# yaricom/Plastic-UNet

Hardware: AMD Instinct MI355X
Metric: training images/sec (128x128, bs=32 per GPU) (higher is better)
Workload: dtype f32; 1 GPU; C2: UNetp depth 5 base_ch 64, oja rule, 1x128x128, fwd+BCE+bwd+Adam; global_batch=32, per_gpu_batch=32, img=128, parallelism=single, step_launch=eager

## Files before the change

### plastic-unet_amd/csrc/common.h

```cpp
#pragma once

#include <hip/hip_runtime.h>
#include <stdint.h>
#include <stdio.h>
#include <stdarg.h>
#include <type_traits>

#include "plastic_unet.h"

namespace pu {

extern thread_local char g_last_error[512];

inline int fail(int code, const char* fmt, ...) {
    va_list ap;
    va_start(ap, fmt);
    vsnprintf(g_last_error, sizeof(g_last_error), fmt, ap);
    va_end(ap);
    return code;
}

inline int check_launch(const char* what) {
    hipError_t e = hipGetLastError();
    if (e != hipSuccess) return fail(PU_ERR_LAUNCH, "%s: %s", what, hipGetErrorString(e));
// ... 76 lines not shown
    return (xcd < r ? xcd * (q + 1) : r * (q + 1) + (xcd - r) * q) + local;
}


template <int N, typename F, int I = 0>
__device__ __forceinline__ void static_for(F&& f) {
    if constexpr (I < N) {
        f(std::integral_constant<int, I>{});
        static_for<N, F, I + 1>(static_cast<F&&>(f));
    }
}
constexpr unsigned LEAN_OOB = 0x80000000u;
typedef __attribute__((address_space(3))) void lds_void_t;

__device__ __forceinline__ void lean_load(const void* base, unsigned bytes, void* lds_dst, unsigned voff, unsigned soff) {
    const unsigned long long b = (unsigned long long)base;
    const unsigned lo = __builtin_amdgcn_readfirstlane((unsigned)b);
    const unsigned hi = __builtin_amdgcn_readfirstlane((unsigned)(b >> 32));
    void* ub = (void*)(((unsigned long long)hi << 32) | lo);
    __amdgpu_buffer_rsrc_t r = __builtin_amdgcn_make_buffer_rsrc(ub, 0, (int)__builtin_amdgcn_readfirstlane(bytes), 0x00020000);
    __builtin_amdgcn_raw_ptr_buffer_load_lds(r, (lds_void_t*)lds_dst, 16, voff, __builtin_amdgcn_readfirstlane(soff), 0, 0);
}

}
```

### plastic-unet_amd/csrc/conv_common.h

```cpp
#pragma once
#include "common.h"

namespace pu {

typedef float f32x4 __attribute__((ext_vector_type(4)));
typedef float f32x16 __attribute__((ext_vector_type(16)));

struct IgemmParams {
    int M, N, K, k_pad;
    int Hi, Wi, Ho, Wo, kh, kw, stride, pad;
    int C, c0, c1;
    const float* src0;
    const float* src1;
    const float* wt;
    const float* bias;
    float* dst0;
    float* dst1;
    const float* mask0;
    const float* mask1;
    int n0, flags;
    int cgroup, taps, gn;
    int vec_epi;
    int ksplit, t_per;
    float* part;
// ... 11 lines not shown
    int oh0, ow0;
    int b;
};

__device__ __forceinline__ EpiRow epi_row(const IgemmParams& p, int m) {
    if (!(p.flags & PU_EPI_SHUFFLE2)) return {m, 0, 0, p.cscale ? (int)fdiv(m, p.dHW) : 0};
    const int t2 = fdiv(m, p.dWo);
    const int wo = m - t2 * p.Wo;
    const int bb = fdiv(t2, p.dHo);
    const int ho = t2 - bb * p.Ho;
    return {(long long)bb * p.shuf_h, 2 * ho - p.shuf_off, 2 * wo - p.shuf_off, bb};
}

__device__ __forceinline__ bool shuf_off(const IgemmParams& p, const EpiRow& r, int n, long long* off, int* c) {
    const int co = p.N >> 2;
    const int ij = fdiv(n, p.dCo);
    *c = n - ij * co;
    const int oh = r.oh0 + (ij >> 1), ow = r.ow0 + (ij & 1);
    if ((unsigned)oh >= (unsigned)p.shuf_h || (unsigned)ow >= (unsigned)p.shuf_w) return false;
    *off = ((r.pix + oh) * p.shuf_w + ow) * co + *c;
    return true;
}

__device__ __forceinline__ void epi_store4(const IgemmParams& p, const EpiRow& r, int n, f32x4 v) {
    float* dst;
    const float* msk;
    long long off;
    int nb;
    const long long pix = r.pix;
    if (p.flags & PU_EPI_SHUFFLE2) {
        if (!shuf_off(p, r, n, &off, &nb)) return;
        dst = p.dst0; msk = p.mask0;
    } else if (n < p.n0) {
        off = pix * p.n0 + n;
        dst = p.dst0; msk = p.mask0; nb = n;
    } else {
        off = pix * (p.N - p.n0) + (n - p.n0);
        dst = p.dst1; msk = p.mask1; nb = n;
    }
    if (p.bias) v += *reinterpret_cast<const f32x4*>(p.bias + nb);
    if (p.resid) v += *reinterpret_cast<const f32x4*>(p.resid + off);
    if (p.flags & PU_EPI_RELU) {
#pragma unroll
        for (int e = 0; e < 4; ++e) v[e] = fmaxf(v[e], 0.f);
    }
    if (msk) {
        const f32x4 mv = *reinterpret_cast<const f32x4*>(msk + off);
#pragma unroll
        for (int e = 0; e < 4; ++e) if (!(mv[e] > 0.f)) v[e] = 0.f;
    }
    if (p.cscale) v *= *reinterpret_cast<const f32x4*>(p.cscale + (long long)r.b * p.cs_ld + nb);
    if (p.flags & PU_EPI_ACCUM) v += *reinterpret_cast<const f32x4*>(dst + off);
    *reinterpret_cast<f32x4*>(dst + off) = v;
}

typedef __bf16 bf16x8_t __attribute__((ext_vector_type(8)));

typedef float f32x2 __attribute__((ext_vector_type(2)));
typedef __bf16 bf16x2_t __attribute__((ext_vector_type(2)));

__device__ __forceinline__ unsigned pk_bf16(f32x2 v) {
    const bf16x2_t h = __builtin_convertvector(v, bf16x2_t);
    return __builtin_bit_cast(unsigned, h);
}

__device__ __forceinline__ void split3_pairs(const f32x4 lo4, const f32x4 hi4, bf16x8_t& h, bf16x8_t& m, bf16x8_t& l) {
#pragma clang fp contract(off)
    typedef unsigned u32x4 __attribute__((ext_vector_type(4)));
    u32x4 hv, mv, lv;
#pragma unroll
    for (int q = 0; q < 4; ++q) {
        const f32x2 x = q < 2 ? f32x2{lo4[2 * q], lo4[2 * q + 1]} : f32x2{hi4[2 * q - 4], hi4[2 * q - 3]};
        const unsigned a = pk_bf16(x);
        const f32x2 af = {__builtin_bit_cast(float, a << 16), __builtin_bit_cast(float, a & 0xffff0000u)};
        const f32x2 r = x - af;
        const unsigned b = pk_bf16(r);
// ... 20 lines not shown
```

### plastic-unet_amd/csrc/elementwise.hip

```cpp
#include "common.h"

#include <math.h>

namespace pu {

typedef float f32x4 __attribute__((ext_vector_type(4)));
typedef __bf16 bf16x4 __attribute__((ext_vector_type(4)));

template <typename T> __device__ __forceinline__ f32x4 ld4(const T* p);
template <> __device__ __forceinline__ f32x4 ld4<float>(const float* p) { return *reinterpret_cast<const f32x4*>(p); }
template <> __device__ __forceinline__ f32x4 ld4<__bf16>(const __bf16* p) {
    const bf16x4 v = *reinterpret_cast<const bf16x4*>(p);
    return f32x4{(float)v[0], (float)v[1], (float)v[2], (float)v[3]};
}
template <typename T> __device__ __forceinline__ void st4(T* p, f32x4 v);
template <> __device__ __forceinline__ void st4<float>(float* p, f32x4 v) { *reinterpret_cast<f32x4*>(p) = v; }
template <> __device__ __forceinline__ void st4<__bf16>(__bf16* p, f32x4 v) {
    *reinterpret_cast<bf16x4*>(p) = bf16x4{(__bf16)v[0], (__bf16)v[1], (__bf16)v[2], (__bf16)v[3]};
}

__device__ __forceinline__ int ungroup_k(int k, int C, int taps, int G) {
    if (G == 0 || k >= taps * C) return k;
    const int tg = k / G, cg = k - tg * G;
    const int g = tg / taps, tap = tg - g * taps;
    return tap * C + g * G + cg;
}

__device__ __forceinline__ float pack_value(const float* __restrict__ w, int mode, int d0, int d1, int taps,
                                            int row, int kc, int G) {
    const int Ck = (mode == PU_PACK_CONV_DGRAD) ? d0 : d1;
    const int k = (mode == PU_PACK_CONVT_FWD) ? kc : ungroup_k(kc, Ck, taps, G);
    float v = 0.f;
    if (mode == PU_PACK_CONV_FWD) {
        if (k < taps * d1) {
            int tap = k / d1, i = k - tap * d1;
            v = w[((long long)row * d1 + i) * taps + tap];
        }
    } else if (mode == PU_PACK_CONV_DGRAD) {
        if (k < taps * d0) {
            int tapf = k / d0, o = k - tapf * d0;
            int tap = taps - 1 - tapf;
// ... 226 lines not shown
    }
}

template <typename T>
struct Vec16 {
    static constexpr int V = 16 / sizeof(T);
    float v[V];
};
template <typename T>
__device__ __forceinline__ Vec16<T> ld16(const T* p) {
    Vec16<T> r;
    if constexpr (sizeof(T) == 4) {
        const f32x4 a = *reinterpret_cast<const f32x4*>(p);
#pragma unroll
        for (int e = 0; e < 4; ++e) r.v[e] = a[e];
    } else {
        typedef __bf16 b8 __attribute__((ext_vector_type(8)));
        const b8 a = *reinterpret_cast<const b8*>(p);
#pragma unroll
        for (int e = 0; e < 8; ++e) r.v[e] = (float)a[e];
    }
    return r;
}
template <typename T>
__device__ __forceinline__ void st16(T* p, const float (&v)[Vec16<T>::V]) {
    if constexpr (sizeof(T) == 4) {
        *reinterpret_cast<f32x4*>(p) = f32x4{v[0], v[1], v[2], v[3]};
    } else {
        typedef __bf16 b8 __attribute__((ext_vector_type(8)));
        b8 a;
#pragma unroll
        for (int e = 0; e < 8; ++e) a[e] = (__bf16)v[e];
        *reinterpret_cast<b8*>(p) = a;
    }
}

template <typename T>
__global__ void maxpool_fwd_win_kernel(const T* __restrict__ x, T* __restrict__ y, int W, int C, int Ho, int Wo,
                                       long long total, const float* __restrict__ scale) {
    constexpr int V = Vec16<T>::V;
    const int CV = C / V;
    for (long long idx = blockIdx.x * (long long)blockDim.x + threadIdx.x; idx < total;
         idx += (long long)gridDim.x * blockDim.x) {
        const int cv = int(idx % CV);
        long long t = idx / CV;
        const int wo = int(t % Wo); t /= Wo;
        const int ho = int(t % Ho);
        const long long b = t / Ho;
        const long long base = (b * 2 * Ho + 2 * ho) * (long long)W + 2 * wo;
        float best[V];
// ... 35 lines not shown
        for (int e = 0; e < V; ++e) { best[e] = -INFINITY; arg[e] = 0; }
#pragma unroll
        for (int q = 0; q < 4; ++q) {
            xv[q] = ld16(x + (base + (q >> 1) * W + (q & 1)) * C + cv * V);
#pragma unroll
            for (int e = 0; e < V; ++e) pool_take(xv[q].v[e], q, best[e], arg[e]);
        }
        Vec16<T> g = ld16(dy + idx * V);
        if (scale) {
#pragma unroll
            for (int e = 0; e < V; ++e) g.v[e] *= scale[b * C + cv * V + e];
        }
#pragma unroll
        for (int q = 0; q < 4; ++q) {
            T* d = dx + (base + (q >> 1) * W + (q & 1)) * C + cv * V;
            float out[V];
#pragma unroll
            for (int e = 0; e < V; ++e) out[e] = (arg[e] == q && (!relu_mask || xv[q].v[e] > 0.f)) ? g.v[e] : 0.f;
            if (accumulate) {
                const Vec16<T> o = ld16(d);
#pragma unroll
                for (int e = 0; e < V; ++e) out[e] = o.v[e] + out[e];
            }
            st16(d, out);
        }
    }
}

template <typename T = float>
__global__ void outconv_fwd_kernel(const T* __restrict__ x, const float* __restrict__ w, const float* __restrict__ b,
                                   float* __restrict__ y, long long rows, int C) {
    const int lane16 = threadIdx.x & 15;
    const long long groups = (long long)gridDim.x * (blockDim.x >> 4);
    const float bias = b ? b[0] : 0.f;
    for (long long m = blockIdx.x * (long long)(blockDim.x >> 4) + (threadIdx.x >> 4); m < rows + 0; m += groups) {
        float s = 0.f;
        for (int c = lane16 * 4; c < C; c += 64) {
            f32x4 v = ld4(x + m * C + c);
            f32x4 ww = *reinterpret_cast<const f32x4*>(w + c);
            s += dot4_fma(v, ww);
        }
        s += __shfl_xor(s, 8, 16);
        s += __shfl_xor(s, 4, 16);
        s += __shfl_xor(s, 2, 16);
        s += __shfl_xor(s, 1, 16);
        if (lane16 == 0) y[m] = s + bias;
    }
// ... 11 lines not shown
constexpr int OC_BLOCKS = 1024;

template <typename T = float>
__global__ void outconv_bwd_kernel(const T* __restrict__ x, const float* __restrict__ w, const float* __restrict__ dy,
                                   T* __restrict__ dx, float* __restrict__ partial, long long rows, int C,
                                   int relu_mask) {
    __shared__ float red[16][65];
    __shared__ float redb[16];
    const int lane16 = threadIdx.x & 15;
    const int grp = threadIdx.x >> 4;
    float* out = partial + (long long)blockIdx.x * (C + 1);
    for (int j = 0; j * 64 < C; ++j) {
        const int c = lane16 * 4 + 64 * j;
        float a0 = 0.f, a1 = 0.f, a2 = 0.f, a3 = 0.f, ab = 0.f;
        for (long long m = blockIdx.x * 16LL + grp; m < rows; m += (long long)gridDim.x * 16) {
            const float g = dy[m];
            ab += g;
            if (c < C) {
                f32x4 v = ld4(x + m * C + c);
                f32x4 ww = *reinterpret_cast<const f32x4*>(w + c);
                f32x4 o;
#pragma unroll
                for (int e = 0; e < 4; ++e) o[e] = (!relu_mask || v[e] > 0.f) ? g * ww[e] : 0.f;
                st4(dx + m * C + c, o);
                a0 += g * v[0]; a1 += g * v[1]; a2 += g * v[2]; a3 += g * v[3];
            }
        }
        __syncthreads();
        red[grp][lane16 * 4 + 0] = a0;
        red[grp][lane16 * 4 + 1] = a1;
        red[grp][lane16 * 4 + 2] = a2;
        red[grp][lane16 * 4 + 3] = a3;
        if (lane16 == 0) redb[grp] = ab;
        __syncthreads();
        const int t = threadIdx.x;
        if (t < 64 && 64 * j + t < C) {
            float s = 0.f;
            for (int q = 0; q < 16; ++q) s += red[q][t];
            out[64 * j + t] = s;
        }
        if (j == 0 && t == 64) {
            float s = 0.f;
            for (int q = 0; q < 16; ++q) s += redb[q];
            out[C] = s;
        }
    }
}
// ... 9 lines not shown
    __shared__ float redb[P];
    const int lane = threadIdx.x % L, grp = threadIdx.x / L;
    const int c = 4 * lane;
    const f32x4 ww = *reinterpret_cast<const f32x4*>(w + c);
    float a0 = 0.f, a1 = 0.f, a2 = 0.f, a3 = 0.f, ab = 0.f;
    const long long stride = (long long)gridDim.x * P;
    for (long long m0 = blockIdx.x * (long long)P + grp; m0 < rows; m0 += OCN_U * stride) {
        f32x4 v[OCN_U];
        float g[OCN_U];
#pragma unroll
        for (int u = 0; u < OCN_U; ++u) {
            const long long m = m0 + u * stride;
            const bool ok = m < rows;
            g[u] = ok ? dy[m] : 0.f;
            v[u] = ok ? ld4(x + m * C + c) : f32x4{0.f, 0.f, 0.f, 0.f};
        }
#pragma unroll
        for (int u = 0; u < OCN_U; ++u) {
            const long long m = m0 + u * stride;
            if (m < rows) {
                f32x4 o;
#pragma unroll
                for (int e = 0; e < 4; ++e) o[e] = (!relu_mask || v[u][e] > 0.f) ? g[u] * ww[e] : 0.f;
                st4(dx + m * C + c, o);
                ab += g[u];
                a0 += g[u] * v[u][0]; a1 += g[u] * v[u][1]; a2 += g[u] * v[u][2]; a3 += g[u] * v[u][3];
            }
        }
    }
    red[grp][c + 0] = a0;
    red[grp][c + 1] = a1;
    red[grp][c + 2] = a2;
    red[grp][c + 3] = a3;
    if (lane == 0) redb[grp] = ab;
    __syncthreads();
    float* out = partial + (long long)blockIdx.x * (C + 1);
    const int t = threadIdx.x;
    if (t < C) {
        float s = 0.f;
        for (int q = 0; q < P; ++q) s += red[q][t];
        out[t] = s;
    } else if (t == C) {
        float s = 0.f;
        for (int q = 0; q < P; ++q) s += redb[q];
        out[C] = s;
    }
}
// ... 524 lines not shown
```

### plastic-unet_amd/csrc/igemm.hip

```cpp
#include "conv_common.h"
#include <type_traits>

namespace pu {


constexpr int IG_BK = 16;
constexpr int IG_LDS = IG_BK + 4;

enum { LOAD_CHUNK16 = 0, LOAD_VEC4 = 1, LOAD_SCALAR = 2 };


template <int MODE>
__device__ __forceinline__ f32x4 load_a4(const IgemmParams& p, int pb, int hb, int wb, int k) {
    f32x4 v = {0.f, 0.f, 0.f, 0.f};
    if (MODE == LOAD_SCALAR) {
#pragma unroll
        for (int e = 0; e < 4; ++e) {
            int ke = k + e;
            if (ke < p.K) {
                int tap = fdiv(ke, p.dC);
                int c = ke - tap * p.C;
                int r = fdiv(tap, p.dKw);
                int s = tap - r * p.kw;
                int hi = hb + r, wi = wb + s;
// ... 3 lines not shown
                }
            }
        }
        return v;
    } else {
        if (k < p.K) {
            int tap = fdiv(k, p.dC);
            int c = k - tap * p.C;
            int r = fdiv(tap, p.dKw);
            int s = tap - r * p.kw;
            int hi = hb + r, wi = wb + s;
            if ((unsigned)hi < (unsigned)p.Hi && (unsigned)wi < (unsigned)p.Wi) {
                long long pix = (long long)pb + hi * p.Wi + wi;
                const float* src = c < p.c0 ? p.src0 + pix * p.c0 + c : p.src1 + pix * p.c1 + (c - p.c0);
                v = *reinterpret_cast<const f32x4*>(src);
            }
        }
        return v;
    }
}


typedef unsigned u32x4_t __attribute__((ext_vector_type(4)));
__device__ __forceinline__ __amdgpu_buffer_rsrc_t epi_rsrc(const void* base, bool on) {
    const unsigned long long b = (unsigned long long)base;
    const unsigned lo = __builtin_amdgcn_readfirstlane((unsigned)b);
    const unsigned hi = __builtin_amdgcn_readfirstlane((unsigned)(b >> 32));
    void* ub = (void*)(((unsigned long long)hi << 32) | lo);
    return __builtin_amdgcn_make_buffer_rsrc(ub, 0, on ? 0x7fffffff : 0, 0x00020000);
}

template <bool MASK, int FM, int FN>
__device__ __forceinline__ void epilogue_batched(const IgemmParams& p, f32x16 (&acc)[FM][FN], int m0, int nc0, int lr,
                                                 int lh) {
    const bool relu = p.flags & PU_EPI_RELU;
    const int n1 = p.N - p.n0;
    unsigned orow[FM][FN];
    bool first[FN];
#pragma unroll
    for (int j = 0; j < FN; ++j) first[j] = nc0 + j * 32 < p.n0;
#pragma unroll
    for (int i = 0; i < FM; ++i) {
        const int m = m0 + i * 32 + lr;
#pragma unroll
        for (int j = 0; j < FN; ++j) {
            const int c = nc0 + j * 32 + 4 * lh - (first[j] ? 0 : p.n0);
// ... 21 lines not shown
    }
#pragma unroll
    for (int j = 0; j < FN; ++j) {
        const __amdgpu_buffer_rsrc_t rd = epi_rsrc(first[j] ? p.dst0 : p.dst1, true);
        const bool has_mk = (first[j] ? p.mask0 : p.mask1) != nullptr;
#pragma unroll
        for (int i = 0; i < FM; ++i)
#pragma unroll
            for (int q = 0; q < 4; ++q) {
                f32x4 v;
#pragma unroll
                for (int e = 0; e < 4; ++e) v[e] = acc[i][j][4 * q + e];
                if constexpr (!MASK) v += ov[0][j][q];
                if (relu) {
#pragma unroll
                    for (int e = 0; e < 4; ++e) v[e] = fmaxf(v[e], 0.f);
                }
                if constexpr (MASK) {
                    if (has_mk) {
#pragma unroll
                        for (int e = 0; e < 4; ++e) if (!(ov[i][j][q][e] > 0.f)) v[e] = 0.f;
                    }
                }
                __builtin_amdgcn_raw_buffer_store_b128(__builtin_bit_cast(u32x4_t, v), rd, orow[i][j], 32 * q, 0);
            }
    }
}

template <int FM, int FN>
__device__ __forceinline__ void epilogue_batched_shuf(const IgemmParams& p, f32x16 (&acc)[FM][FN], int m0, int nc0,
                                                      int lr, int lh) {
    const bool relu = p.flags & PU_EPI_RELU;
    const int co = p.N >> 2;
    unsigned orow[FM][FN];
    int cj[FN];
#pragma unroll
    for (int j = 0; j < FN; ++j) {
        const int nj = nc0 + j * 32;
        const int ij = nj < p.N ? nj / co : 0;
        cj[j] = nj - ij * co + 4 * lh;
#pragma unroll
        for (int i = 0; i < FM; ++i) {
            const int m = m0 + i * 32 + lr;
            unsigned o = LEAN_OOB;
            if (m < p.M && nj < p.N) {
                const int t2 = fdiv(m, p.dWo);
                const int wo = m - t2 * p.Wo;
// ... 8 lines not shown
    f32x4 bv[FN][4];
    const __amdgpu_buffer_rsrc_t rb = epi_rsrc(p.bias, true);
#pragma unroll
    for (int j = 0; j < FN; ++j)
#pragma unroll
        for (int q = 0; q < 4; ++q)
            bv[j][q] = __builtin_bit_cast(f32x4, __builtin_amdgcn_raw_buffer_load_b128(
                rb, nc0 + j * 32 < p.N ? (unsigned)cj[j] * 4u : LEAN_OOB, 32 * q, 0));
    const __amdgpu_buffer_rsrc_t rd = epi_rsrc(p.dst0, true);
#pragma unroll
    for (int j = 0; j < FN; ++j)
#pragma unroll
        for (int i = 0; i < FM; ++i)
#pragma unroll
            for (int q = 0; q < 4; ++q) {
                f32x4 v;
#pragma unroll
                for (int e = 0; e < 4; ++e) v[e] = acc[i][j][4 * q + e];
                v += bv[j][q];
                if (relu) {
#pragma unroll
                    for (int e = 0; e < 4; ++e) v[e] = fmaxf(v[e], 0.f);
                }
                __builtin_amdgcn_raw_buffer_store_b128(__builtin_bit_cast(u32x4_t, v), rd, orow[i][j], 32 * q, 0);
            }
}

template <int BM, int BN, int WM, int WN, bool BATCH = false>
__device__ __forceinline__ void epilogue(const IgemmParams& p, f32x16 (&acc)[BM / WM / 32][BN / WN / 32], int m_blk,
                                         int n_blk, int wm, int wn, int lr, int lh) {
    constexpr int FM = BM / WM / 32;
    constexpr int FN = BN / WN / 32;
    if constexpr (BATCH) {
        if (p.vec_epi && !(p.flags & (PU_EPI_SHUFFLE2 | PU_EPI_ACCUM)) && !p.resid && !p.cscale && p.n0 % 32 == 0 &&
            p.N % 32 == 0 && (long long)p.M * p.N < (1LL << 29)) {
            const int m0 = m_blk + wm * (BM / WM), nc0 = n_blk + wn * (BN / WN);
            if ((p.mask0 || p.mask1) && !p.bias) {
                epilogue_batched<true, FM, FN>(p, acc, m0, nc0, lr, lh);
                return;
            }
            if (!p.mask0 && !p.mask1 && p.bias) {
                epilogue_batched<false, FM, FN>(p, acc, m0, nc0, lr, lh);
                return;
            }
        }
        if (p.vec_epi && (p.flags & PU_EPI_SHUFFLE2) && !(p.flags & PU_EPI_ACCUM) && !p.resid && !p.cscale && p.bias &&
            !p.mask0 && p.shuf_off == 0 && p.shuf_h == 2 * p.Ho && p.shuf_w == 2 * p.Wo && (p.N / 4) % 32 == 0 &&
// ... 349 lines not shown
        }
        __builtin_amdgcn_sched_group_barrier(0x100, 2 * (FM + FN), 0);
        __builtin_amdgcn_sched_group_barrier(0x008, 8 * FM * FN, 0);
    }
    asm volatile("s_waitcnt vmcnt(0)" ::: "memory");
    if (p.ksplit == 1) {
        epilogue<BM, BN, WM, WN>(p, acc, m_blk, n_blk, wm, wn, lr, lh);
        return;
    }
    float* part = p.part + (long long)kz * p.M * p.N;
#pragma unroll
    for (int i = 0; i < FM; ++i) {
        const int m = m_blk + wm * (BM / WM) + i * 32 + lr;
        if (m >= p.M) continue;
#pragma unroll
        for (int j = 0; j < FN; ++j)
#pragma unroll
            for (int q = 0; q < 4; ++q) {
                const int n = n_blk + wn * (BN / WN) + j * 32 + 8 * q + 4 * lh;
                if (n >= p.N) continue;
                f32x4 v;
#pragma unroll
                for (int e = 0; e < 4; ++e) v[e] = acc[i][j][4 * q + e];
                *reinterpret_cast<f32x4*>(part + (long long)m * p.N + n) = v;
            }
    }
}


__device__ __forceinline__ void split3_bf16(const f32x4 lo4, const f32x4 hi4, bf16x8_t& h, bf16x8_t& m, bf16x8_t& l) {
#pragma clang fp contract(off)
#pragma unroll
    for (int e = 0; e < 8; ++e) {
        const float x = e < 4 ? lo4[e] : hi4[e - 4];
        const __bf16 a = (__bf16)x;
        const float r = x - (float)a;
        const __bf16 b = (__bf16)r;
        const float q = r - (float)b;
        h[e] = a;
        m[e] = b;
        l[e] = (__bf16)q;
    }
}

template <int BM, int BN, int WM, int WN, int NW = 4>
__global__ __launch_bounds__(NW * 64) void igemm_x6_kernel(const IgemmParams p) {
    constexpr int NBUF = 3;
// ... 148 lines not shown
            }
            if (i == 0) issue(ts + NBUF - 1, (ts + NBUF - 1) % NBUF);
        }
    }
    asm volatile("s_waitcnt vmcnt(0)" ::: "memory");
    if (p.ksplit == 1) {
        epilogue<BM, BN, WM, WN, true>(p, acc, m_blk, n_blk, wm, wn, lr, lh);
        return;
    }
    float* part = p.part + (long long)kz * p.M * p.N;
#pragma unroll
    for (int i = 0; i < FM; ++i) {
        const int m = m_blk + wm * (BM / WM) + i * 32 + lr;
        if (m >= p.M) continue;
#pragma unroll
        for (int j = 0; j < FN; ++j)
#pragma unroll
            for (int q = 0; q < 4; ++q) {
                const int n = n_blk + wn * (BN / WN) + j * 32 + 8 * q + 4 * lh;
                if (n >= p.N) continue;
                f32x4 v;
#pragma unroll
                for (int e = 0; e < 4; ++e) v[e] = acc[i][j][4 * q + e];
                *reinterpret_cast<f32x4*>(part + (long long)m * p.N + n) = v;
            }
    }
}


template <int BM, int BN, int WM, int WN, int NW, int CG>
__global__ __launch_bounds__(NW * 64) void igemm_x6_lean_kernel(const IgemmParams p) {
    constexpr int FM = BM / WM / 32;
    constexpr int FN = BN / WN / 32;
    constexpr int A_LD = BM / (16 * NW);
    constexpr int W_TOT = 6 * BN / 64;
    constexpr int W_LD = (W_TOT + NW - 1) / NW;
    constexpr bool SINK = (W_TOT % NW) != 0;
    constexpr int G = A_LD + W_LD;
    constexpr int A_FL = BM * 16;
    constexpr int W_FL = BN * 6 * 4;
    constexpr int STAGE = A_FL + W_FL;
    constexpr int SPG = 9 * CG;
    static_assert(WM * WN == NW && A_LD >= 1 && SPG % 3 == 0, "lean tile");

    __shared__ __attribute__((aligned(16))) float lds[3 * STAGE + (SINK ? 256 : 0)];

    const int tid = threadIdx.x;
// ... 144 lines not shown
                }
            }
        });
    }
    asm volatile("s_waitcnt vmcnt(0)" ::: "memory");
    if (p.ksplit == 1) {
        epilogue<BM, BN, WM, WN, true>(p, acc, m_blk, n_blk, wm, wn, lr, lh);
        return;
    }
    float* part = p.part + (long long)kz * p.M * p.N;
#pragma unroll
    for (int i = 0; i < FM; ++i) {
        const int m = m_blk + wm * (BM / WM) + i * 32 + lr;
        if (m >= p.M) continue;
#pragma unroll
        for (int j = 0; j < FN; ++j)
#pragma unroll
            for (int q = 0; q < 4; ++q) {
                const int n = n_blk + wn * (BN / WN) + j * 32 + 8 * q + 4 * lh;
                if (n >= p.N) continue;
                f32x4 v;
#pragma unroll
                for (int e = 0; e < 4; ++e) v[e] = acc[i][j][4 * q + e];
                *reinterpret_cast<f32x4*>(part + (long long)m * p.N + n) = v;
            }
    }
}

__global__ void split_weight6_kernel(const float* __restrict__ w, __bf16* __restrict__ out, int n, int k_pad) {
#pragma clang fp contract(off)
    const long long total = (long long)n * k_pad;
    for (long long idx = blockIdx.x * 256LL + threadIdx.x; idx < total; idx += (long long)gridDim.x * 256) {
        const int row = (int)(idx / k_pad);
        const int k = (int)(idx - (long long)row * k_pad);
        const float x = w[idx];
        const __bf16 a = (__bf16)x;
        const float r = x - (float)a;
        const __bf16 b = (__bf16)r;
        const __bf16 c = (__bf16)(r - (float)b);
        const int t = k >> 4, half = (k >> 3) & 1, e = k & 7;
        const __bf16 v[3] = {a, b, c};
#pragma unroll
        for (int pl = 0; pl < 3; ++pl)
            out[(((long long)t * 6 + pl * 2 + half) * n + row) * 8 + e] = v[pl];
    }
}

__global__ __launch_bounds__(256) void igemm_splitk_epilogue_kernel(const IgemmParams p) {
    const int nq = p.N >> 2;
    const long long idx = (long long)blockIdx.x * 256 + threadIdx.x;
    if (idx >= (long long)p.M * nq) return;
    const int m = (int)(idx / nq);
    const int n = (int)(idx - (long long)m * nq) * 4;
    const long long mn = (long long)p.M * p.N;
    const float* src = p.part + (long long)m * p.N + n;
    f32x4 v = *reinterpret_cast<const f32x4*>(src);
    for (int z = 1; z < p.ksplit; ++z) v += *reinterpret_cast<const f32x4*>(src + z * mn);
    epi_store4(p, epi_row(p, m), n, v);
}

constexpr int SC_TH = 16, SC_TW = 32;

template <int C, int N, int KP = (9 * C + 15) / 16 * 16>
__global__ __launch_bounds__(256) void smallconv_kernel(const IgemmParams p) {
    constexpr int HH = SC_TH + 2, HWD = SC_TW + 2;
    constexpr int CP = (C + 3) & ~3;
    __shared__ __attribute__((aligned(16))) float tile[HH * HWD * CP];
    const int tiles_w = (p.Wo + SC_TW - 1) / SC_TW;
    const int tiles_h = (p.Ho + SC_TH - 1) / SC_TH;
    int blk = blockIdx.x;
    const int txi = blk % tiles_w;
    blk /= tiles_w;
    const int tyi = blk % tiles_h;
    const int b = blk / tiles_h;
    const int y0 = tyi * SC_TH - 1, x0 = txi * SC_TW - 1;
    const long long img = (long long)b * p.Hi * p.Wi;

    if (C % 4 == 0 && p.c0 % 4 == 0) {
        constexpr int Q = C / 4 > 0 ? C / 4 : 1;
        constexpr int NE = HH * HWD * Q;
        constexpr int PT = (NE + 255) / 256;
// ... 540 lines not shown
```

### plastic-unet_amd/csrc/wgrad.hip

```cpp
#include "common.h"
#include <type_traits>

#ifndef PU_NO_ILV
#define PU_NO_ILV 0
#endif
#ifndef PU_WW_ABL
#define PU_WW_ABL 0
#endif

namespace pu {

typedef float f32x4 __attribute__((ext_vector_type(4)));
typedef float f32x16 __attribute__((ext_vector_type(16)));

constexpr int WG_BM = 16;

struct WgradParams {
    int M, N, Nr, K, Kc, C, c0, c1;
    int Hi, Wi, Ho, Wo, kw, stride, pad;
    const float* P;
    const float* src0;
    const float* src1;
    int bias_mode;
    float* slab;
    int mps;
    int gx, gy;
    int Kcp;
    int batch, tiles_w, tiles_h;
    FastDiv dWo, dHo, dC, dKw;
};

template <int BN, int BK, int WN, int WK, bool QVEC>
__global__ __launch_bounds__(256) void wgrad_kernel(const WgradParams p) {
    constexpr int FN = BN / WN / 32;
    constexpr int FK = BK / WK / 32;
    constexpr int P_PER_ROW = BN / 4;
    constexpr int P_LD = (WG_BM * P_PER_ROW) / 256;
    constexpr int Q_PER_ROW = BK / 4;
// ... 413 lines not shown
    float* slab = p.slab + (long long)tz * p.Nr * p.Kcp;
    if (tid < bias_w) {
        if (p.bias_mode == 1) {
            const int n = n_blk + tid;
            if (n < p.N) slab[(long long)n * p.Kcp + p.K] = bsum;
        } else {
            const int k = k_blk + tid;
            if (k < p.K) slab[(long long)p.N * p.Kcp + k] = bsum;
        }
    }
#pragma unroll
    for (int j = 0; j < FN; ++j) {
        const int n = n_blk + wn * (BN / WN) + j * 32 + lr;
        if (n >= p.N) continue;
#pragma unroll
        for (int i = 0; i < FK; ++i) {
#pragma unroll
            for (int q = 0; q < 4; ++q) {
                const int k = k_blk + wk * (BK / WK) + i * 32 + 8 * q + 4 * lh;
                if (k >= p.K) continue;
                f32x4 v;
#pragma unroll
                for (int e = 0; e < 4; ++e) v[e] = acc[i][j][4 * q + e];
                *reinterpret_cast<f32x4*>(slab + (long long)n * p.Kcp + k) = v;
            }
        }
    }
}

typedef short wi16x4 __attribute__((ext_vector_type(4)));
typedef __attribute__((address_space(3))) wi16x4 lds_i16x4_t;
__device__ __forceinline__ int wb_sw(int r) { return ((r & 3) << 2) | ((r >> 2) & 3); }

constexpr int HX_ROWS = 54;
constexpr int HX_IMG = (HX_ROWS + 16) * 128;
__device__ __forceinline__ int hx_off(int row, int col) {
    return row * 128 + 16 * ((col >> 3) ^ (((row >> 1) & 1) << 2)) + 2 * (col & 7);
}

template <int NT>
__global__ __launch_bounds__(256 * NT) void wgrad_halo_x6_kernel(const WgradParams p) {
    constexpr int NTH = 256 * NT;
    constexpr int RS = NTH / 16;
    constexpr int XG = (HX_ROWS + RS - 1) / RS;
    constexpr int IMG = (HX_ROWS + 16 * NT) * 128;
    __shared__ __attribute__((aligned(16))) char lds[2 * 3 * IMG];

// ... 423 lines not shown

    decode_x(0);
    load_x(0);
    load_x(1);
    load_x(2);
    load_x(3);
    decode_g(0);
    load_g(0);
    load_g(1);
    form(std::integral_constant<int, 0>{}, lx0, lg0);
    decode_x(1);
    load_x(0);
    asm volatile("s_waitcnt lgkmcnt(0)" ::: "memory");
    __builtin_amdgcn_s_barrier();
    asm volatile("" ::: "memory");
    for (int k = 0; k < S; ++k) {
        sub(k, std::integral_constant<int, 0>{});
        sub(k, std::integral_constant<int, 1>{});
        sub(k, std::integral_constant<int, 2>{});
        sub(k, std::integral_constant<int, 3>{});
    }
    asm volatile("s_waitcnt vmcnt(0) lgkmcnt(0)" ::: "memory");

    float* slab = p.slab + (long long)z * p.Nr * p.Kcp;
    if (p.bias_mode == 1 && cx == 0) {
        wg_f32x2* red = reinterpret_cast<wg_f32x2*>(lg0);
        red[tid] = bsum;
        __syncthreads();
        if (tid < 32) {
            wg_f32x2 v = red[tid];
            for (int r = 1; r < 16; ++r) v += red[r * 32 + tid];
            slab[(long long)(ny * 64 + 2 * tid) * p.Kcp + p.K] = v[0];
            slab[(long long)(ny * 64 + 2 * tid + 1) * p.Kcp + p.K] = v[1];
        }
        __syncthreads();
    }

    const float sj1 = wj ? -1.f : 1.f;
    float* xs = reinterpret_cast<float*>(wc ? lx1 : lx0) + (wn * 2 + wj) * 24 * 64;
    const float* xrd = reinterpret_cast<const float*>(wc ? lx1 : lx0) + (wn * 2 + (1 - wj)) * 24 * 64;
    const int lr = lane & 31, lh = lane >> 5;
    const int n = ny * 64 + wn * 32 + lr;
#pragma unroll
    for (int r = 0; r < 3; ++r) {
        float mine[2][3][4], other[2][3][4];
#pragma unroll
        for (int q = 0; q < 4; ++q)
#pragma unroll
            for (int ee = 0; ee < 4; ++ee) {
                const int idx = 4 * q + ee;
                float R[2];
#pragma unroll
                for (int jj = 0; jj < 2; ++jj) {
                    const float m0 = acc[0 * 2 + jj][idx], m1 = acc[1 * 2 + jj][idx];
                    const float m2 = acc[2 * 2 + jj][idx], m3 = -acc[3 * 2 + jj][idx];
                    float v = r == 0 ? m0 + 0.5f * (m1 + m2) : r == 1 ? 0.5f * (m1 - m2) : 0.5f * (m1 + m2) + m3;
// ... 15 lines not shown
                    if (keep) mine[q & 1][s][ee] = P[s];
                    else other[q & 1][s][ee] = P[s];
                }
            }
#pragma unroll
        for (int qh = 0; qh < 2; ++qh)
#pragma unroll
            for (int s = 0; s < 3; ++s)
#pragma unroll
                for (int ee = 0; ee < 4; ++ee) xs[((qh * 3 + s) * 4 + ee) * 64 + lane] = other[qh][s][ee];
        __syncthreads();
#pragma unroll
        for (int qh = 0; qh < 2; ++qh)
#pragma unroll
            for (int s = 0; s < 3; ++s) {
                f32x4 v;
#pragma unroll
                for (int ee = 0; ee < 4; ++ee) {
                    const float o = xrd[((qh * 3 + s) * 4 + ee) * 64 + lane];
                    v[ee] = wj == 0 ? mine[qh][s][ee] + o : o + mine[qh][s][ee];
                }
                const int q = 2 * wj + qh;
                const int k = (3 * r + s) * p.C + c_lo + wc * 32 + 8 * q + 4 * lh;
                *reinterpret_cast<f32x4*>(slab + (long long)n * p.Kcp + k) = v;
            }
        __syncthreads();
    }
}

constexpr int SWS_TH = 16, SWS_TW = 64;

template <int N, bool BF16ROWS = false>
__global__ __launch_bounds__(256) void wgrad_stem_kernel(const WgradParams p) {
    constexpr int L = N / 4, PG = 256 / L;
    constexpr int HH = SWS_TH + 2, HW = SWS_TW + 2;
    constexpr int RED = PG * 10 * N;
    __shared__ __attribute__((aligned(16))) float smem[RED > HH * HW ? RED : HH * HW];
    const int tid = threadIdx.x;
    const int lane_c = tid % L, grp = tid / L;
    float acc[10][4];
#pragma unroll
    for (int k = 0; k < 10; ++k)
#pragma unroll
        for (int e = 0; e < 4; ++e) acc[k][e] = 0.f;
    const int ntiles = p.batch * p.tiles_h * p.tiles_w;
    for (int t = blockIdx.x; t < ntiles; t += gridDim.x) {
        const int txi = t % p.tiles_w;
// ... 348 lines not shown

__device__ __forceinline__ void store_oihw(int n, int k, float v, int K, int C, int kh, int kw, int bias_mode,
                                           float* __restrict__ dw, float* __restrict__ db, int accumulate) {
    if (k < K) {
        const int tap = k / C, c = k - tap * C;
        const int r = tap / kw, ss = tap - r * kw;
        float* o = dw + (((long long)n * C + c) * kh + r) * kw + ss;
        *o = accumulate ? *o + v : v;
    } else if (bias_mode == 1 && k == K) {
        db[n] = accumulate ? db[n] + v : v;
    }
}

__global__ __launch_bounds__(256) void wgrad_sum_splits4_kernel(const float* __restrict__ slab, int splits,
                                                                long long total, int G, double* __restrict__ part) {
    const long long idx = 4 * (blockIdx.x * (long long)blockDim.x + threadIdx.x);
    if (idx >= total) return;
    const int g = blockIdx.y;
    const f64x4 s = sum_chains<8>(reinterpret_cast<const f32x4*>(slab + (long long)g * total + idx),
                                  (splits - g + G - 1) / G, G * (total >> 2));
    double* o = part + (long long)g * total + idx;
#pragma unroll
    for (int e = 0; e < 4; ++e) o[e] = s[e];
}

template <typename T>
__global__ __launch_bounds__(256) void wgrad_finish4_kernel(const T* __restrict__ part, int G, int Nr, int Kc, int N,
                                                            int K, int C, int kh, int kw, int bias_mode,
                                                            float* __restrict__ dw, float* __restrict__ db,
                                                            int accumulate) {
    typedef T t4 __attribute__((ext_vector_type(4)));
    const long long total = (long long)Nr * Kc;
    const long long nq = total >> 2;
    const long long q = blockIdx.x * (long long)blockDim.x + threadIdx.x;
    if (q < nq) {
        const long long idx = 4 * q;
        const int n = int(idx / Kc);
        const int k0 = int(idx - (long long)n * Kc);
        if (n >= N) return;
        const f64x4 s = sum_chains<8>(reinterpret_cast<const t4*>(part + idx), G, nq);
#pragma unroll
        for (int e = 0; e < 4; ++e) store_oihw(n, k0 + e, (float)s[e], K, C, kh, kw, bias_mode, dw, db, accumulate);
    } else if (bias_mode == 2 && q < nq + C) {
        const int c = int(q - nq);
        const int J = kh * kw * G;
        const T* bp = part + (long long)N * Kc + c;
// ... 626 lines not shown
    if (transposed) {
        hipLaunchKernelGGL(wgrad_finish_t_kernel<T>, dim3((unsigned)ceil_div(pl.C, 256), (unsigned)a->n),
                           dim3((unsigned)(64 * taps)), 0, s, part, count, pl.Nr, pl.Kcp, pl.K, pl.C, taps, a->bias_mode,
                           a->dweight, a->dbias, a->accumulate);
        return;
    }
    const long long threads = (long long)pl.Nr * pl.Kcp / 4 + (a->bias_mode == 2 ? pl.C : 0);
    hipLaunchKernelGGL(wgrad_finish4_kernel<T>, dim3((unsigned)((threads + 255) / 256)), dim3(256), 0, s, part, count,
                       pl.Nr, pl.Kcp, a->n, pl.K, pl.C, a->kh, a->kw, a->bias_mode, a->dweight, a->dbias, a->accumulate);
}

constexpr long long WR_WIDE_MAX = 16384;

static int wgrad_reduce(const WgradPlan& pl, const pu_wgrad_args* a, void* workspace, hipStream_t s) {
    const long long total = (long long)pl.Nr * pl.Kcp;
    const float* slab = (const float*)workspace;
    if ((pl.small || pl.stem || pl.pw || (!pl.wino && total <= WR_WIDE_MAX)) && a->bias_mode != 2) {
        hipLaunchKernelGGL(wgrad_reduce_wide_kernel, dim3((unsigned)ceil_div(total, (long long)WR_E)), dim3(256), 0, s,
                           slab, pl.splits, total, a->n, pl.Kcp, pl.K, pl.C, a->kh, a->kw, a->bias_mode, a->dweight,
                           a->dbias, a->accumulate);
        return check_launch("pu_wgrad (reduce)");
    }
    const bool transposed = a->bias_mode != 2 && a->kh * a->kw <= 9 && pl.C % 4 == 0 && ((uintptr_t)a->dweight & 15) == 0;
    if (pl.G > 1) {
        double* part = (double*)((char*)workspace + ((pl.slab_bytes() + 255) / 256) * 256);
        hipLaunchKernelGGL(wgrad_sum_splits4_kernel, dim3((unsigned)((total / 4 + 255) / 256), pl.G), dim3(256), 0, s,
                           slab, pl.splits, total, pl.G, part);
        launch_finisher(transposed, (const double*)part, pl.G, pl, a, s);
    } else {
        launch_finisher(transposed, slab, pl.splits, pl, a, s);
    }
    return check_launch("pu_wgrad (reduce)");
}

static int plan_wgrad_bf16(const pu_wgrad_args* a, WgradPlan* pl) {
    PU_REQUIRE(a && a->batch > 0 && a->out_h > 0 && a->out_w > 0 && a->in_h > 0 && a->in_w > 0, "pu_wgrad_bf16: bad grid");
    PU_REQUIRE(a->kh > 0 && a->kw > 0 && a->stride > 0 && a->pad >= 0, "pu_wgrad_bf16: bad taps");
    PU_REQUIRE(a->rows && a->n > 0 && a->src0 && a->c0 > 0 && (a->c1 == 0 || a->src1), "pu_wgrad_bf16: operands");
    PU_REQUIRE(a->n % 8 == 0 && a->c0 % 8 == 0 && a->c1 % 8 == 0,
               "pu_wgrad_bf16: n (%d) and channel counts (%d, %d) must be multiples of 8", a->n, a->c0, a->c1);
    PU_REQUIRE(a->bias_mode >= 0 && a->bias_mode <= 2 && (a->bias_mode == 0 || a->dbias) && a->dweight, "pu_wgrad_bf16: outputs");
    PU_REQUIRE((((uintptr_t)a->rows | (uintptr_t)a->src0 | (uintptr_t)a->src1) & 15) == 0, "pu_wgrad_bf16: 16-byte alignment");
    if (int st = plan_dims(a, pl, "pu_wgrad_bf16")) return st;
    const long long M = pl->M;
    pl->qvec = true; pl->dma = true; pl->small = false; pl->stem = false;
    pl->halo = false;
    if (a->kh == 3 && a->kw == 3 && a->stride == 1 && a->pad == 1 && a->in_h == a->out_h &&
// ... 207 lines not shown
```

### plastic-unet_amd/csrc/winograd.hip

```cpp
#include "conv_common.h"

#ifndef PU_NO_ILV
#define PU_NO_ILV 0
#endif

namespace pu {

typedef unsigned u32x2 __attribute__((ext_vector_type(2)));
typedef unsigned u32x4 __attribute__((ext_vector_type(4)));

constexpr int WG_BM = 64;
constexpr int WG_BN = 64;
constexpr int WG_WIDE_BM = 32;
constexpr int WG_WIDE_BN = 128;

struct WinoParams {
    IgemmParams p;
    const __bf16* U;
    int tiles;
    int kc_per;
    int gm;
    FastDiv dTw, dTh;
    unsigned a_bytes;
    unsigned u_bytes;
};

__device__ __forceinline__ __amdgpu_buffer_rsrc_t uniform_rsrc(const void* base, unsigned bytes) {
    const unsigned long long b = (unsigned long long)base;
    const unsigned lo = __builtin_amdgcn_readfirstlane((unsigned)b);
    const unsigned hi = __builtin_amdgcn_readfirstlane((unsigned)(b >> 32));
    void* ub = (void*)(((unsigned long long)hi << 32) | lo);
    return __builtin_amdgcn_make_buffer_rsrc(ub, 0, (int)__builtin_amdgcn_readfirstlane(bytes), 0x00020000);
}

__device__ __forceinline__ f32x4 epi_ld4(__amdgpu_buffer_rsrc_t r, unsigned off) {
    return __builtin_bit_cast(f32x4, __builtin_amdgcn_raw_buffer_load_b128(r, off, 0, 0));
}
__device__ __forceinline__ void epi_st4(__amdgpu_buffer_rsrc_t r, unsigned off, f32x4 v) {
    __builtin_amdgcn_raw_buffer_store_b128(__builtin_bit_cast(u32x4, v), r, off, 0, 0);
}

#ifndef PU_W4_ABL
#define PU_W4_ABL 0
#endif
#ifndef PU_W4_VA
#define PU_W4_VA 2
#endif
#ifndef PU_W4_ITEM_STAMP
#define PU_W4_ITEM_STAMP 0
#endif
#if PU_W4_ITEM_STAMP
constexpr int PU_W4_NBLK = 4096;
__device__ unsigned long long pu_w4_item_buf[PU_W4_NBLK * 8];
__device__ __forceinline__ void w4_item_stamp(int k, unsigned long long v) {
    if (threadIdx.x == 0 && blockIdx.x < PU_W4_NBLK) pu_w4_item_buf[blockIdx.x * 8 + k] = v;
}
#define W4S(k) w4_item_stamp(k, __builtin_amdgcn_s_memtime())
#else
#define W4S(k) ((void)0)
#endif
constexpr int W4_VH = 4 * 3 * 64 * 32;
constexpr int W4_XF = 4 * 2 * 16 * 64;
#ifndef PU_W4_XCH1
// ... 429 lines not shown
                for (int g = 0; g < 4; ++g)
#pragma unroll
                    for (int o = 0; o < 2; ++o) mv[g][o] = epi_ld4(r_msk, o_px + py * o_row + o * o_col + 32u * g);
#pragma unroll
                for (int g = 0; g < 4; ++g) {
                    asm volatile("" :: "v"(bv[g]));
#pragma unroll
                    for (int o = 0; o < 2; ++o) asm volatile("" :: "v"(mv[g][o]));
                }
#pragma unroll
                for (int g = 0; g < 4; ++g)
#pragma unroll
                    for (int o = 0; o < 2; ++o) {
                        f32x4 v = yv(py, o, g);
                        if (p.bias) v += bv[g];
                        if (relu) {
#pragma unroll
                            for (int e = 0; e < 4; ++e) v[e] = fmaxf(v[e], 0.f);
                        }
                        if (msk) {
#pragma unroll
                            for (int e = 0; e < 4; ++e) if (!(mv[g][o][e] > 0.f)) v[e] = 0.f;
                        }
                        epi_st4(r_dst, o_px + py * o_row + o * o_col + 32u * g, v);
                    }
            }
        } else {
            const __amdgpu_buffer_rsrc_t r_acc = uniform_rsrc(dst, accum ? RANGE : 0u);
            const __amdgpu_buffer_rsrc_t r_res = uniform_rsrc(p.resid, p.resid ? RANGE : 0u);
            const __amdgpu_buffer_rsrc_t r_cs = uniform_rsrc(p.cscale, p.cscale ? RANGE : 0u);
            const unsigned o_cs = (unsigned)(b * p.cs_ld + e_n) * 4u;
#pragma unroll
            for (int py = 0; py < 2; ++py) {
                f32x4 bv[4], sv4[4], rv[4][2], mv[4][2], av[4][2];
#pragma unroll
                for (int g = 0; g < 4; ++g) {
                    bv[g] = epi_ld4(r_bias, (unsigned)(e_n + 8 * g) * 4u);
                    sv4[g] = epi_ld4(r_cs, o_cs + 32u * g);
#pragma unroll
                    for (int o = 0; o < 2; ++o) {
                        const unsigned off = o_px + py * o_row + o * o_col + 32u * g;
                        rv[g][o] = epi_ld4(r_res, off);
                        mv[g][o] = epi_ld4(r_msk, off);
                        av[g][o] = epi_ld4(r_acc, off);
                    }
                }
#pragma unroll
                for (int g = 0; g < 4; ++g) {
                    asm volatile("" :: "v"(bv[g]), "v"(sv4[g]));
#pragma unroll
                    for (int o = 0; o < 2; ++o) asm volatile("" :: "v"(rv[g][o]), "v"(mv[g][o]), "v"(av[g][o]));
                }
#pragma unroll
                for (int g = 0; g < 4; ++g)
#pragma unroll
                    for (int o = 0; o < 2; ++o) {
                        f32x4 v = yv(py, o, g);
                        if (p.bias) v += bv[g];
                        if (p.resid) v += rv[g][o];
                        if (relu) {
#pragma unroll
                            for (int e = 0; e < 4; ++e) v[e] = fmaxf(v[e], 0.f);
                        }
                        if (msk) {
#pragma unroll
                            for (int e = 0; e < 4; ++e) if (!(mv[g][o][e] > 0.f)) v[e] = 0.f;
                        }
                        if (p.cscale) v *= sv4[g];
                        if (accum) v += av[g][o];
                        epi_st4(r_dst, o_px + py * o_row + o * o_col + 32u * g, v);
                    }
            }
        }
    } else if (e_ok) {
        float* part = p.part + (long long)kz * p.M * p.N + pix00 * p.N + e_n;
#pragma unroll
        for (int py = 0; py < 2; ++py)
#pragma unroll
            for (int o = 0; o < 2; ++o)
#pragma unroll
                for (int g = 0; g < 4; ++g)
                    *reinterpret_cast<f32x4*>(part + ((long long)py * p.Wo + o) * p.N + 8 * g) = yv(py, o, g);
    }
    W4S(4);
    asm volatile("s_waitcnt vmcnt(0)" ::: "memory");
    W4S(5);
}

struct WinoPackJob {
    const float* w;
    __bf16* out;
    int n, c, dgrad, blocks;
};
constexpr int WINO_MAX_JOBS = 64;
struct WinoPackBatch {
    WinoPackJob job[WINO_MAX_JOBS];
    int count;
};

constexpr int WP_N = 32, WP_C = 64;
constexpr int WP_LD = WP_C * 9 + 1;
__global__ __launch_bounds__(256) void wino_pack_kernel(const WinoPackBatch bt) {
#pragma clang fp contract(off)
    __shared__ float gw[WP_N * WP_LD];
    int j = 0, b0 = 0;
// ... 205 lines not shown
```

Before: 4764 images/s.

## Add per-kernel store cache policies and fused grouped wgrad split-sum finish kernel

Introduces a templated store-policy layer (plain vs write-through sc1 stores, plus buffer-store variants) and threads it through conv epilogues, split-K partial writes, maxpool backward and outconv backward stores. Write-through is enabled by default for maxpool backward and the split-K reduce epilogue, to change how those outputs are placed in the cache hierarchy for the consumers that follow. It also adds a single-kernel finish for grouped wgrad split reduction (G≤16, no bias_mode 2) that sums partial slabs in double in shared memory and writes OIHW directly, replacing the two-pass partial-sum path. The inline asm store with s_nop and the double-precision reduction may add latency.

```diff
diff --git a/plastic-unet_amd/csrc/common.h b/plastic-unet_amd/csrc/common.h
--- a/plastic-unet_amd/csrc/common.h
+++ b/plastic-unet_amd/csrc/common.h
@@ -122,4 +122,33 @@
     __builtin_amdgcn_raw_ptr_buffer_load_lds(r, (lds_void_t*)lds_dst, 16, voff, __builtin_amdgcn_readfirstlane(soff), 0, 0);
 }
 
+constexpr int ST_PLAIN = 0;
+constexpr int ST_WT = 16;
+
+typedef float f32x4 __attribute__((ext_vector_type(4)));
+
+__device__ __forceinline__ __amdgpu_buffer_rsrc_t st_rsrc(const void* base, unsigned bytes) {
+    const unsigned long long b = (unsigned long long)base;
+    const unsigned lo = __builtin_amdgcn_readfirstlane((unsigned)b);
+    const unsigned hi = __builtin_amdgcn_readfirstlane((unsigned)(b >> 32));
+    void* ub = (void*)(((unsigned long long)hi << 32) | lo);
+    return __builtin_amdgcn_make_buffer_rsrc(ub, 0, (int)__builtin_amdgcn_readfirstlane(bytes), 0x00020000);
 }
+template <int POLICY>
+__device__ __forceinline__ void st_buf4(__amdgpu_buffer_rsrc_t r, unsigned voff, unsigned soff, f32x4 v) {
+    typedef unsigned u4 __attribute__((ext_vector_type(4)));
+    __builtin_amdgcn_raw_buffer_store_b128(__builtin_bit_cast(u4, v), r, voff, soff, POLICY);
+}
+template <int POLICY>
+__device__ __forceinline__ void st_buf1(__amdgpu_buffer_rsrc_t r, unsigned voff, unsigned soff, float v) {
+    __builtin_amdgcn_raw_buffer_store_b32(__builtin_bit_cast(unsigned, v), r, voff, soff, POLICY);
+}
+template <int POLICY>
+__device__ __forceinline__ void st_glb4(void* p, f32x4 v) {
+    if constexpr (POLICY == ST_WT)
+        asm volatile("global_store_dwordx4 %0, %1, off sc1\n\ts_nop 1" ::"v"(p), "v"(v) : "memory");
+    else
+        *reinterpret_cast<f32x4*>(p) = v;
+}
+
+}
diff --git a/plastic-unet_amd/csrc/conv_common.h b/plastic-unet_amd/csrc/conv_common.h
--- a/plastic-unet_amd/csrc/conv_common.h
+++ b/plastic-unet_amd/csrc/conv_common.h
@@ -57,6 +57,7 @@
     return true;
 }
 
+template <int POLICY = ST_PLAIN>
 __device__ __forceinline__ void epi_store4(const IgemmParams& p, const EpiRow& r, int n, f32x4 v) {
     float* dst;
     const float* msk;
@@ -86,7 +87,7 @@
     }
     if (p.cscale) v *= *reinterpret_cast<const f32x4*>(p.cscale + (long long)r.b * p.cs_ld + nb);
     if (p.flags & PU_EPI_ACCUM) v += *reinterpret_cast<const f32x4*>(dst + off);
-    *reinterpret_cast<f32x4*>(dst + off) = v;
+    st_glb4<POLICY>(dst + off, v);
 }
 
 typedef __bf16 bf16x8_t __attribute__((ext_vector_type(8)));
diff --git a/plastic-unet_amd/csrc/elementwise.hip b/plastic-unet_amd/csrc/elementwise.hip
--- a/plastic-unet_amd/csrc/elementwise.hip
+++ b/plastic-unet_amd/csrc/elementwise.hip
@@ -17,6 +17,17 @@
 template <> __device__ __forceinline__ void st4<float>(float* p, f32x4 v) { *reinterpret_cast<f32x4*>(p) = v; }
 template <> __device__ __forceinline__ void st4<__bf16>(__bf16* p, f32x4 v) {
     *reinterpret_cast<bf16x4*>(p) = bf16x4{(__bf16)v[0], (__bf16)v[1], (__bf16)v[2], (__bf16)v[3]};
+}
+
+#ifndef PU_ST_MAXPOOL_BWD
+#define PU_ST_MAXPOOL_BWD ST_WT
+#endif
+#ifndef PU_ST_OUTCONV_BWD
+#define PU_ST_OUTCONV_BWD ST_PLAIN
+#endif
+template <int POLICY, typename T> __device__ __forceinline__ void st4_end(T* p, f32x4 v) {
+    if constexpr (sizeof(T) == 4) st_glb4<POLICY>(p, v);
+    else st4(p, v);
 }
 
 __device__ __forceinline__ int ungroup_k(int k, int C, int taps, int G) {
@@ -289,10 +300,10 @@
     }
     return r;
 }
-template <typename T>
+template <typename T, int POLICY = ST_PLAIN>
 __device__ __forceinline__ void st16(T* p, const float (&v)[Vec16<T>::V]) {
     if constexpr (sizeof(T) == 4) {
-        *reinterpret_cast<f32x4*>(p) = f32x4{v[0], v[1], v[2], v[3]};
+        st_glb4<POLICY>(p, f32x4{v[0], v[1], v[2], v[3]});
     } else {
         typedef __bf16 b8 __attribute__((ext_vector_type(8)));
         b8 a;
@@ -374,7 +385,7 @@
 #pragma unroll
                 for (int e = 0; e < V; ++e) out[e] = o.v[e] + out[e];
             }
-            st16(d, out);
+            st16<T, PU_ST_MAXPOOL_BWD>(d, out);
         }
     }
 }
@@ -432,7 +443,7 @@
                 f32x4 o;
 #pragma unroll
                 for (int e = 0; e < 4; ++e) o[e] = (!relu_mask || v[e] > 0.f) ? g * ww[e] : 0.f;
-                st4(dx + m * C + c, o);
+                st4_end<PU_ST_OUTCONV_BWD>(dx + m * C + c, o);
                 a0 += g * v[0]; a1 += g * v[1]; a2 += g * v[2]; a3 += g * v[3];
             }
         }
@@ -488,7 +499,7 @@
                 f32x4 o;
 #pragma unroll
                 for (int e = 0; e < 4; ++e) o[e] = (!relu_mask || v[u][e] > 0.f) ? g[u] * ww[e] : 0.f;
-                st4(dx + m * C + c, o);
+                st4_end<PU_ST_OUTCONV_BWD>(dx + m * C + c, o);
                 ab += g[u];
                 a0 += g[u] * v[u][0]; a1 += g[u] * v[u][1]; a2 += g[u] * v[u][2]; a3 += g[u] * v[u][3];
             }
diff --git a/plastic-unet_amd/csrc/igemm.hip b/plastic-unet_amd/csrc/igemm.hip
--- a/plastic-unet_amd/csrc/igemm.hip
+++ b/plastic-unet_amd/csrc/igemm.hip
@@ -49,6 +49,15 @@
 
 
 typedef unsigned u32x4_t __attribute__((ext_vector_type(4)));
+#ifndef PU_ST_IGEMM_EPI
+#define PU_ST_IGEMM_EPI ST_PLAIN
+#endif
+#ifndef PU_ST_IGEMM_PART
+#define PU_ST_IGEMM_PART ST_PLAIN
+#endif
+#ifndef PU_ST_SPLITK_EPI
+#define PU_ST_SPLITK_EPI ST_WT
+#endif
 __device__ __forceinline__ __amdgpu_buffer_rsrc_t epi_rsrc(const void* base, bool on) {
     const unsigned long long b = (unsigned long long)base;
     const unsigned lo = __builtin_amdgcn_readfirstlane((unsigned)b);
@@ -116,7 +125,7 @@
                         for (int e = 0; e < 4; ++e) if (!(ov[i][j][q][e] > 0.f)) v[e] = 0.f;
                     }
                 }
-                __builtin_amdgcn_raw_buffer_store_b128(__builtin_bit_cast(u32x4_t, v), rd, orow[i][j], 32 * q, 0);
+                st_buf4<PU_ST_IGEMM_EPI>(rd, orow[i][j], 32 * q, v);
             }
     }
 }
@@ -171,7 +180,7 @@
 #pragma unroll
                     for (int e = 0; e < 4; ++e) v[e] = fmaxf(v[e], 0.f);
                 }
-                __builtin_amdgcn_raw_buffer_store_b128(__builtin_bit_cast(u32x4_t, v), rd, orow[i][j], 32 * q, 0);
+                st_buf4<PU_ST_IGEMM_EPI>(rd, orow[i][j], 32 * q, v);
             }
 }
 
@@ -567,7 +576,7 @@
                 f32x4 v;
 #pragma unroll
                 for (int e = 0; e < 4; ++e) v[e] = acc[i][j][4 * q + e];
-                *reinterpret_cast<f32x4*>(part + (long long)m * p.N + n) = v;
+                st_glb4<PU_ST_IGEMM_PART>(part + (long long)m * p.N + n, v);
             }
     }
 }
@@ -762,7 +771,7 @@
                 f32x4 v;
 #pragma unroll
                 for (int e = 0; e < 4; ++e) v[e] = acc[i][j][4 * q + e];
-                *reinterpret_cast<f32x4*>(part + (long long)m * p.N + n) = v;
+                st_glb4<PU_ST_IGEMM_PART>(part + (long long)m * p.N + n, v);
             }
     }
 }
@@ -953,7 +962,7 @@
                 f32x4 v;
 #pragma unroll
                 for (int e = 0; e < 4; ++e) v[e] = acc[i][j][4 * q + e];
-                *reinterpret_cast<f32x4*>(part + (long long)m * p.N + n) = v;
+                st_glb4<PU_ST_IGEMM_PART>(part + (long long)m * p.N + n, v);
             }
     }
 }
@@ -987,7 +996,7 @@
     const float* src = p.part + (long long)m * p.N + n;
     f32x4 v = *reinterpret_cast<const f32x4*>(src);
     for (int z = 1; z < p.ksplit; ++z) v += *reinterpret_cast<const f32x4*>(src + z * mn);
-    epi_store4(p, epi_row(p, m), n, v);
+    epi_store4<PU_ST_SPLITK_EPI>(p, epi_row(p, m), n, v);
 }
 
 constexpr int SC_TH = 16, SC_TW = 32;
diff --git a/plastic-unet_amd/csrc/wgrad.hip b/plastic-unet_amd/csrc/wgrad.hip
--- a/plastic-unet_amd/csrc/wgrad.hip
+++ b/plastic-unet_amd/csrc/wgrad.hip
@@ -14,6 +14,13 @@
 typedef float f32x16 __attribute__((ext_vector_type(16)));
 
 constexpr int WG_BM = 16;
+
+#ifndef PU_ST_WGRAD_WINO
+#define PU_ST_WGRAD_WINO ST_PLAIN
+#endif
+#ifndef PU_ST_WGRAD_DMA
+#define PU_ST_WGRAD_DMA ST_PLAIN
+#endif
 
 struct WgradParams {
     int M, N, Nr, K, Kc, C, c0, c1;
@@ -473,7 +480,7 @@
                 f32x4 v;
 #pragma unroll
                 for (int e = 0; e < 4; ++e) v[e] = acc[i][j][4 * q + e];
-                *reinterpret_cast<f32x4*>(slab + (long long)n * p.Kcp + k) = v;
+                st_glb4<PU_ST_WGRAD_DMA>(slab + (long long)n * p.Kcp + k, v);
             }
         }
     }
@@ -943,7 +950,8 @@
     }
     asm volatile("s_waitcnt vmcnt(0) lgkmcnt(0)" ::: "memory");
 
-    float* slab = p.slab + (long long)z * p.Nr * p.Kcp;
+    const __amdgpu_buffer_rsrc_t r_slab =
+        ww_rsrc(p.slab + (long long)z * p.Nr * p.Kcp, (unsigned)p.Nr * (unsigned)p.Kcp * 4u);
     if (p.bias_mode == 1 && cx == 0) {
         wg_f32x2* red = reinterpret_cast<wg_f32x2*>(lg0);
         red[tid] = bsum;
@@ -951,8 +959,8 @@
         if (tid < 32) {
             wg_f32x2 v = red[tid];
             for (int r = 1; r < 16; ++r) v += red[r * 32 + tid];
-            slab[(long long)(ny * 64 + 2 * tid) * p.Kcp + p.K] = v[0];
-            slab[(long long)(ny * 64 + 2 * tid + 1) * p.Kcp + p.K] = v[1];
+            st_buf1<PU_ST_WGRAD_WINO>(r_slab, (unsigned)((ny * 64 + 2 * tid) * p.Kcp + p.K) * 4u, 0, v[0]);
+            st_buf1<PU_ST_WGRAD_WINO>(r_slab, (unsigned)((ny * 64 + 2 * tid + 1) * p.Kcp + p.K) * 4u, 0, v[1]);
         }
         __syncthreads();
     }
@@ -1014,7 +1022,7 @@
                 }
                 const int q = 2 * wj + qh;
                 const int k = (3 * r + s) * p.C + c_lo + wc * 32 + 8 * q + 4 * lh;
-                *reinterpret_cast<f32x4*>(slab + (long long)n * p.Kcp + k) = v;
+                st_buf4<PU_ST_WGRAD_WINO>(r_slab, (unsigned)(n * p.Kcp + k) * 4u, 0, v);
             }
         __syncthreads();
     }
@@ -1409,6 +1417,27 @@
     double* o = part + (long long)g * total + idx;
 #pragma unroll
     for (int e = 0; e < 4; ++e) o[e] = s[e];
+}
+
+template <int QB>
+__global__ __launch_bounds__(512) void wgrad_sum_finish_kernel(const float* __restrict__ slab, int splits,
+                                                               long long total, int G, int N, int Kcp, int K, int C,
+                                                               int kh, int kw, int bias_mode, float* __restrict__ dw,
+                                                               float* __restrict__ db, int accumulate) {
+    __shared__ f64x4 part[512 / QB][QB];
+    const int q = threadIdx.x, g = threadIdx.y;
+    const long long idx = 4 * (blockIdx.x * (long long)QB + q);
+    if (idx < total)
+        part[g][q] = sum_chains<8>(reinterpret_cast<const f32x4*>(slab + (long long)g * total + idx),
+                                   (splits - g + G - 1) / G, G * (total >> 2));
+    __syncthreads();
+    if (g != 0 || idx >= total) return;
+    const f64x4 s = sum_chains<4>(&part[0][q], G, (long long)QB);
+    const int n = int(idx / Kcp);
+    const int k0 = int(idx - (long long)n * Kcp);
+    if (n >= N) return;
+#pragma unroll
+    for (int e = 0; e < 4; ++e) store_oihw(n, k0 + e, (float)s[e], K, C, kh, kw, bias_mode, dw, db, accumulate);
 }
 
 template <typename T>
@@ -2081,7 +2110,17 @@
         return check_launch("pu_wgrad (reduce)");
     }
     const bool transposed = a->bias_mode != 2 && a->kh * a->kw <= 9 && pl.C % 4 == 0 && ((uintptr_t)a->dweight & 15) == 0;
-    if (pl.G > 1) {
+    if (pl.G > 1 && pl.G <= 16 && a->bias_mode != 2) {
+        const long long nq = total / 4;
+        if (pl.G <= 8)
+            hipLaunchKernelGGL(wgrad_sum_finish_kernel<64>, dim3((unsigned)ceil_div(nq, 64LL)), dim3(64, (unsigned)pl.G), 0,
+                               s, slab, pl.splits, total, pl.G, a->n, pl.Kcp, pl.K, pl.C, a->kh, a->kw, a->bias_mode,
+                               a->dweight, a->dbias, a->accumulate);
+        else
+            hipLaunchKernelGGL(wgrad_sum_finish_kernel<32>, dim3((unsigned)ceil_div(nq, 32LL)), dim3(32, (unsigned)pl.G), 0,
+                               s, slab, pl.splits, total, pl.G, a->n, pl.Kcp, pl.K, pl.C, a->kh, a->kw, a->bias_mode,
+                               a->dweight, a->dbias, a->accumulate);
+    } else if (pl.G > 1) {
         double* part = (double*)((char*)workspace + ((pl.slab_bytes() + 255) / 256) * 256);
         hipLaunchKernelGGL(wgrad_sum_splits4_kernel, dim3((unsigned)((total / 4 + 255) / 256), pl.G), dim3(256), 0, s,
                            slab, pl.splits, total, pl.G, part);
diff --git a/plastic-unet_amd/csrc/winograd.hip b/plastic-unet_amd/csrc/winograd.hip
--- a/plastic-unet_amd/csrc/winograd.hip
+++ b/plastic-unet_amd/csrc/winograd.hip
@@ -36,9 +36,16 @@
 __device__ __forceinline__ f32x4 epi_ld4(__amdgpu_buffer_rsrc_t r, unsigned off) {
     return __builtin_bit_cast(f32x4, __builtin_amdgcn_raw_buffer_load_b128(r, off, 0, 0));
 }
+template <int POLICY>
 __device__ __forceinline__ void epi_st4(__amdgpu_buffer_rsrc_t r, unsigned off, f32x4 v) {
-    __builtin_amdgcn_raw_buffer_store_b128(__builtin_bit_cast(u32x4, v), r, off, 0, 0);
-}
+    st_buf4<POLICY>(r, off, 0, v);
+}
+#ifndef PU_ST_W4_EPI
+#define PU_ST_W4_EPI ST_PLAIN
+#endif
+#ifndef PU_ST_W4_PART
+#define PU_ST_W4_PART ST_PLAIN
+#endif
 
 #ifndef PU_W4_ABL
 #define PU_W4_ABL 0
@@ -514,7 +521,7 @@
 #pragma unroll
                             for (int e = 0; e < 4; ++e) if (!(mv[g][o][e] > 0.f)) v[e] = 0.f;
                         }
-                        epi_st4(r_dst, o_px + py * o_row + o * o_col + 32u * g, v);
+                        epi_st4<PU_ST_W4_EPI>(r_dst, o_px + py * o_row + o * o_col + 32u * g, v);
                     }
             }
         } else {
@@ -560,7 +567,7 @@
                         }
                         if (p.cscale) v *= sv4[g];
                         if (accum) v += av[g][o];
-                        epi_st4(r_dst, o_px + py * o_row + o * o_col + 32u * g, v);
+                        epi_st4<PU_ST_W4_EPI>(r_dst, o_px + py * o_row + o * o_col + 32u * g, v);
                     }
             }
         }
@@ -572,7 +579,7 @@
             for (int o = 0; o < 2; ++o)
 #pragma unroll
                 for (int g = 0; g < 4; ++g)
-                    *reinterpret_cast<f32x4*>(part + ((long long)py * p.Wo + o) * p.N + 8 * g) = yv(py, o, g);
+                    st_glb4<PU_ST_W4_PART>(part + ((long long)py * p.Wo + o) * p.N + 8 * g, yv(py, o, g));
     }
     W4S(4);
     asm volatile("s_waitcnt vmcnt(0)" ::: "memory");
```

Result: no change. 4781 images/s (median of 6 runs) (+0.4%).
